# innnky/vispeech

Measured on AMD Instinct MI355X. Metric: 44.1kHz samples/sec, higher is better.
Workload: dtype f32 (split-f16 MFMA, 3-term); 1 GPU; C3: 64 mixed zh/ja utterances (~5 s each) per GPU, 44.1 kHz, hop 512, phoneme/duration/F0/energy/noise supplied, random-init (synthetic) weights of configs/config.json; 2 batches in flight per GPU; utterances_per_gpu=64, global_batch=64, padded_frames=489, frames_padded=31296, frames_computed=28902, parallelism=shard1, generator=f16s, controls=all, batches_in_flight=2

## Files before the change

vispeech_amd/csrc/api.hip:

```cpp
#include <algorithm>
#include <cmath>
#include <cstdlib>
#include <cstring>
#include <vector>

#include "model.h"

using namespace vsp;

namespace {

void generator_frame_dependence(const vsp_config& c, int resblock, int pre_k, int post_k, int& back, int& fwd);
long total_upsample(const vsp_config& c);

struct T3 {
  float* p = nullptr;
  long bs = 0, cs = 0;
  T3 chan(int c) const { return T3{p ? p + (size_t)c * cs : nullptr, bs, cs}; }
};

struct Ws {
  char* base;
  size_t cap;
  size_t cur = 0;
// ... 142 lines not shown
    if (prof) {
      const double in_el = (double)a.T_in * a.Cin, out_el = (double)(a.ups_s > 0 ? a.T_store * (a.M / a.ups_s) : a.Nq * a.M);
      const double ext = 4.0 * B * (in_el + out_el * (1.0 + (a.res ? 1.0 : 0.0) + (a.acc_prev ? 1.0 : 0.0)));
      prof_end(cls, 2.0 * a.M * a.Cin * a.K * (double)a.Nq * B, 4.0 * B * (in_el + out_el), ext, ext);
    }
  }
  void clconv(const ClConv& L, const float* x, float* out, const float* res, int T, bool acc_prev, float div, int B,
              const uint16_t* x_img = nullptr, uint16_t* o_img = nullptr) {
    if (dry() || !ok()) return;
    ClConvArgs a = L.phases > 1 ? cl_ups_args(cw(L), L.Cin, L.Cout, L.K, L.phases, x, T, CL_LRELU_SLOPE, out, terms())
                                : cl_conv_args(cw(L), L.Cin, L.Cout, L.K, L.dil, x, T, CL_LRELU_SLOPE, res, out, terms());
    a.x_img = x_img; a.o_img = o_img;
    a.acc_prev = acc_prev ? 1 : 0; a.div = div;
    a.glen = glen; a.g_in = L.phases > 1 ? grate_in : grate_out; a.g_store = grate_out;
    const bool prof = prof_begin(VSP_PROF_GENERATOR, fam(L.phases > 1 ? VSP_FAM_UPS : VSP_FAM_CONV, L.Cout));
    chk(launch_g16_conv(a, B, s), "g16_conv");
    if (prof) {
      const double in_el = (double)a.T_in * L.Cin, out_el = (double)a.T_store * L.Cout;
      const double ext = 4.0 * B * (in_el + out_el * (1.0 + (res ? 1.0 : 0.0) + (acc_prev ? 1.0 : 0.0)));
      prof_end(VSP_PROF_GENERATOR, 2.0 * L.Cout * L.Cin * L.K * L.phases * (double)a.Nq * B, 4.0 * B * (in_el + out_el), ext,
               ext + (out && o_img ? 4.0 * B * out_el : 0.0));
    }
  }
  void cond(const Conv& L, const float* g, float* out, int B) {
    const int gin = L.Cin;
    ConvArgs a = args(L, T3{const_cast<float*>(g), (long)gin, 1}, T3{out, (long)L.M, 1}, 1, 1);
    conv(a, B);
  }
  void ln(T3 x, T3 res, size_t gamma, size_t beta, T3 y, int B, int C, int T) {
    if (dry() || !ok()) return;
    chk(launch_layernorm(x.p, x.bs, x.cs, res.p, res.bs, res.cs, A(gamma), A(beta), y.p, y.bs, y.cs, B, C, T, s),
        "layernorm");
  }
};

void run_encoder_masked(Run& r, const EncoderW& E, int B, int T, T3 x_in, const int64_t* lengths, T3 y_out) {
  const vsp_config& c = r.ctx->cfg;
  const int h = c.hidden_channels, f = c.filter_channels;
  T3 X = r.ws.t3(B, h, T), S = r.ws.t3(B, h, T), QKV = r.ws.t3(B, 3 * h, T), AT = r.ws.t3(B, h, T),
     FF = r.ws.t3(B, f, T);
  void* AP = r.ctx->att_f16s ? r.ws.bytes(3 * attn_pack_bytes(B, c.n_heads, h / c.n_heads, T)) : nullptr;
  if (E.layers.empty()) {
    if (!r.dry() && r.ok()) {
      r.chk(launch_copy3(x_in.p, x_in.bs, x_in.cs, y_out.p, y_out.bs, y_out.cs, B, h, T, r.s), "copy");
      if (lengths) r.chk(launch_mask3(y_out.p, y_out.bs, y_out.cs, lengths, B, h, T, r.s), "mask");
    }
// ... 44 lines not shown
        }
      }
    } else {
      r.conv(a, B);
      r.ln(S, T3{}, L.g1, L.b1, X, B, h, T);
    }
    a = r.args(L.f1, X, FF, T, T);
    a.lengths = lengths; a.in_mask = 1; a.act = 1;
    r.conv(a, B);
    a = r.args(L.f2, FF, S, T, T);
    a.lengths = lengths; a.in_mask = 1; a.mask_pre = 1;
    a.res = X.p; a.r_bs = X.bs; a.r_cs = X.cs;
    r.conv(a, B);
    r.ln(S, T3{}, L.g2, L.b2, last ? y_out : X, B, h, T);
  }
  if (lengths && !r.dry() && r.ok()) r.chk(launch_mask3(y_out.p, y_out.bs, y_out.cs, lengths, B, h, T, r.s), "mask");
}

void mask3(Run& r, T3 x, const int64_t* lengths, int B, int C, int T) {
  if (r.dry() || !r.ok() || !lengths) return;
  r.chk(launch_mask3(x.p, x.bs, x.cs, lengths, B, C, T, r.s), "mask");
}

void run_wn(Run& r, const Conv* cond, const std::vector<Conv>& in, const std::vector<Conv>& res,
            const std::vector<Conv>& skip, int nl, int B, int T, T3 H, T3 ACT, T3 OUT, float* gc, long gc_bs, const float* g,
            const int64_t* lengths) {
  const int h = r.ctx->cfg.hidden_channels;
  if (cond) r.cond(*cond, g, gc, B);
  for (int l = 0; l < nl; ++l) {
    ConvArgs a = r.args(in[l], H, ACT, T, T);
    a.act = 2; a.cond = gc ? gc + (size_t)l * 2 * h : nullptr; a.cond_bs = gc_bs;
    r.conv(a, B);
    if (l < nl - 1) {
      a = r.args(res[l], ACT, H, T, T);
      a.res = H.p; a.r_bs = H.bs; a.r_cs = H.cs;
      a.lengths = lengths; a.mask_post = 1;
      a.split_row = h; a.out2 = OUT.p; a.o2_bs = OUT.bs; a.o2_cs = OUT.cs; a.acc_prev2 = l > 0;
      r.conv(a, B);
    } else {
      a = r.args(skip[l], ACT, OUT, T, T);
      a.acc_prev = l > 0;
      a.lengths = lengths; a.mask_post = 1;
      r.conv(a, B);
    }
  }
}

void run_flow(Run& r, int B, int T, T3 z, const float* g, const int64_t* lengths, bool reverse = true) {
  const vsp_config& c = r.ctx->cfg;
  const Model& m = r.ctx->model;
  const int h = c.hidden_channels, half = c.inter_channels / 2, fl = c.flow_layers;
  T3 H = r.ws.t3(B, h, T), ACT = r.ws.t3(B, h, T), OUT = r.ws.t3(B, h, T);
  const long gcs = (long)c.n_flows * 2 * h * fl;
  float* gc = r.ws.f((size_t)B * gcs);
  r.cond(m.flow_cond_all, g, gc, B);
  for (int n = 0; n < c.n_flows; ++n) {
    const int i = reverse ? c.n_flows - 1 - n : n;
    const FlowW& F = m.flows[i];
    const T3 x0 = F.flipped ? z.chan(half) : z;
    const T3 x1 = F.flipped ? z : z.chan(half);
    ConvArgs a = r.args(F.pre, x0, H, T, T);
    a.lengths = lengths; a.mask_post = 1;
    r.conv(a, B);
    run_wn(r, nullptr, F.in, F.res, F.skip, fl, B, T, H, ACT, OUT, gc ? gc + (size_t)i * 2 * h * fl : nullptr, gcs, g, lengths);
    a = r.args(F.post, OUT, x1, T, T);
    a.lengths = lengths; a.mask_pre = 1; a.alpha = reverse ? -1.f : 1.f;
    a.res = x1.p; a.r_bs = x1.bs; a.r_cs = x1.cs;
    a.mask_post = 1;
    r.conv(a, B);
  }
}

void run_posterior(Run& r, int B, int T, T3 y, const int64_t* lengths, const float* g, const float* noise, T3 Z,
                   T3 M, T3 LOGS) {
  const vsp_config& c = r.ctx->cfg;
  const PosteriorW& Q = r.ctx->model.enc_q;
  const int h = c.hidden_channels, ql = c.posterior_layers;
  T3 H = r.ws.t3(B, h, T), ACT = r.ws.t3(B, h, T), OUT = r.ws.t3(B, h, T);
  float* gc = r.ws.f((size_t)B * 2 * h * ql);
  if (r.dry()) return;
  ConvArgs a = r.args(Q.pre, y, H, T, T);
  a.lengths = lengths; a.mask_post = 1;
  r.conv(a, B);
  run_wn(r, &Q.cond, Q.in, Q.res, Q.skip, ql, B, T, H, ACT, OUT, gc, 2L * h * ql, g, lengths);
  a = r.args(Q.proj, OUT, M, T, T);
  a.lengths = lengths; a.mask_post = 1;
  a.split_row = c.inter_channels; a.out2 = LOGS.p; a.o2_bs = LOGS.bs; a.o2_cs = LOGS.cs; a.mask_post2 = 1;
  r.conv(a, B);
  if (r.ok()) {
    r.chk(launch_reparam(M.p, LOGS.p, noise, 1.f, Z.p, (long)B * c.inter_channels * T, r.s), "reparam");
    r.chk(launch_mask3(Z.p, Z.bs, Z.cs, lengths, B, c.inter_channels, T, r.s), "mask");
  }
}

template <class F>
size_t max_over_stages(const vsp_config& c, int T, size_t mx, F f) {
  long t = T;
  for (int i = 0; i < c.n_upsamples; ++i) {
    t *= c.upsample_rates[i];
    mx = std::max(mx, (size_t)f(c.upsample_initial_channel >> (i + 1), t));
  }
  return mx;
}

void run_generator(Run& r, int B, int T, T3 z, const int64_t* in_lengths, const float* g, float* o) {
  const vsp_config& c = r.ctx->cfg;
  const Model& m = r.ctx->model;
// ... 335 lines not shown
  if (!cfg || !out || (resblock != 1 && resblock != 2)) return VSP_ERR_ARG;
  vsp_ctx* ctx = new (std::nothrow) vsp_ctx();
  if (!ctx) return VSP_ERR_ARG;
  ctx->cfg = *cfg;
  ctx->resblock = resblock;
  ctx->device = device;
  if (const char* e = getenv("VSP_FRAME")) ctx->frame_f16s = strcmp(e, "f32") != 0;
  if (const char* e = getenv("VSP_ATT")) ctx->att_f16s = strcmp(e, "f32") != 0;
  bool want_f16 = false;
  if (const char* e = getenv("VSP_GENERATOR")) {
    if (!strcmp(e, "f32")) ctx->gen_mode = 0;
    want_f16 = !strcmp(e, "f16");
  }
  if (const char* e = getenv("VSP_FUSE_PAIRS")) ctx->fuse_pairs = atoi(e) != 0;
  if (const char* e = getenv("VSP_RB2_FUSE")) ctx->rb2_fuse = atoi(e) != 0;
  if (const char* e = getenv("VSP_TIMG")) ctx->t_img = atoi(e) != 0;
  if (const char* e = getenv("VSP_PP")) ctx->pp_pairs = atoi(e) != 0;
  if (const char* e = getenv("VSP_PAIR")) ctx->pair_ring = !strcmp(e, "ring");
  if (const char* e = getenv("VSP_CHAIN_RING")) ctx->chain_ring = atoi(e) != 0;
  if (const char* e = getenv("VSP_CHAIN")) ctx->chain_mask = atoi(e);
  if (const char* e = getenv("VSP_RW64")) ctx->rw64 = atoi(e) != 0;
  if (const char* e = getenv("VSP_TRIM_TAILS")) ctx->trim_tails = atoi(e) != 0;
  if (const char* e = getenv("VSP_COLS")) ctx->cols = atoi(e) != 0;
  if (const char* e = getenv("VSP_COLS_BLOCKS")) ctx->cols_blocks = atol(e);
  if (const char* e = getenv("VSP_COLS_MIN_BLOCKS")) ctx->cols_min_blocks = atol(e);
  if (const char* e = getenv("VSP_ACT_SCALE_LOG2")) {
    const int l = atoi(e);
    ctx->act_scale = std::ldexp(1.f, l < 0 ? 0 : l > 8 ? 8 : l);
  }
  if (const char* e = getenv("VSP_EARLY_FL")) ctx->early_fl = atoi(e) != 0;
  if (const char* e = getenv("VSP_RB_STREAMS")) ctx->rb_streams = atoi(e);
#ifdef VSP_EXPERIMENTS
  if (const char* e = getenv("VSP_ATT_KSPLIT")) ctx->att_ksplit = atoi(e);
  if (const char* e = getenv("VSP_CHUNK_MB")) ctx->chunk_mb = atof(e);
  if (const char* e = getenv("VSP_CHAIN_CH")) ctx->chain_ch = atoi(e);
  if (const char* e = getenv("VSP_CHAIN128")) ctx->chain128_mask = atoi(e);
#endif
  build_schema(ctx->cfg, ctx->schema, ctx->resblock);
  const int rc = plan_model(ctx);
  if (want_f16 && ctx->gen_mode == 1) ctx->gen_mode = 2;
  *out = ctx;
  return rc;
}

int vsp_destroy(vsp_ctx* ctx) {
  if (!ctx) return VSP_ERR_ARG;
// ... 615 lines not shown
  Run r{ctx, (hipStream_t)stream, ws};
  const long n = (long)B * ctx->cfg.inter_channels * Tf;
  r.chk(hipMemcpyAsync(z_p, z, n * sizeof(float), hipMemcpyDeviceToDevice, r.s), "z copy");
  run_flow(r, B, Tf, ext(z_p, ctx->cfg.inter_channels, Tf), g, frame_lengths, false);
  if (ws.overflow) return ctx->fail(VSP_ERR_WORKSPACE, "flow workspace too small (need %zu bytes)", ws.cur);
  return r.rc;
}

static int check_vc(vsp_ctx* ctx);

static int wn_layer_impl(vsp_ctx* ctx, hipStream_t s, Ws& ws, int which, int layer, int B, int T, float* x, const float* g,
                         const int64_t* lengths, float* skip, int accumulate) {
  const vsp_config& c = ctx->cfg;
  const Model& m = ctx->model;
  const int h = c.hidden_channels;
  const bool post = which < 0;
  const Conv& cond = post ? m.enc_q.cond : m.flows[which].cond;
  const std::vector<Conv>& in = post ? m.enc_q.in : m.flows[which].in;
  const std::vector<Conv>& res = post ? m.enc_q.res : m.flows[which].res;
  const std::vector<Conv>& sk = post ? m.enc_q.skip : m.flows[which].skip;
  const int nl = post ? c.posterior_layers : c.flow_layers;
  Run r{ctx, s, ws};
  T3 ACT = ws.t3(B, h, T);
  float* gc = ws.f((size_t)B * 2 * h * nl);
  if (ws.dry) return VSP_OK;
  if (ws.overflow) return ctx->fail(VSP_ERR_WORKSPACE, "wn layer workspace too small");
  const T3 H = ext(x, h, T), OUT = ext(skip, h, T);
  r.cond(cond, g, gc, B);
  ConvArgs a = r.args(in[layer], H, ACT, T, T);
  a.act = 2; a.cond = gc + (size_t)layer * 2 * h; a.cond_bs = 2L * h * nl;
  r.conv(a, B);
  if (layer < nl - 1) {
    a = r.args(res[layer], ACT, H, T, T);
    a.res = H.p; a.r_bs = H.bs; a.r_cs = H.cs;
    a.lengths = lengths; a.mask_post = 1;
    a.split_row = h; a.out2 = OUT.p; a.o2_bs = OUT.bs; a.o2_cs = OUT.cs; a.acc_prev2 = accumulate ? 1 : 0;
    r.conv(a, B);
  } else {
    a = r.args(sk[layer], ACT, OUT, T, T);
    a.acc_prev = accumulate ? 1 : 0;
    a.lengths = lengths; a.mask_post = 1;
    r.conv(a, B);
  }
  return r.rc;
}

int64_t vsp_wn_layer_workspace_bytes(const vsp_ctx* ctx, int which, int B, int T) {
  if (!ctx || B <= 0 || T <= 0 || which < -1 || which >= ctx->cfg.n_flows) return VSP_ERR_ARG;
  if (which < 0 && ctx->cfg.spec_channels <= 0) return VSP_ERR_ARG;
  Ws ws(nullptr, 0, true);
  wn_layer_impl(const_cast<vsp_ctx*>(ctx), nullptr, ws, which, 0, B, T, nullptr, nullptr, nullptr, nullptr, 0);
// ... 408 lines not shown
```

vispeech_amd/csrc/kernels.h:

```cpp
#pragma once
#include <hip/hip_runtime.h>
#include <stdint.h>

#include <atomic>

#include "../../include/vispeech_hip.h"

namespace vsp {

inline hipError_t set_max_dynamic_lds(const void* kern, int bytes, std::atomic<uint64_t>& done) {
  int dev = 0;
  hipError_t e = hipGetDevice(&dev);
  if (e != hipSuccess) return e;
  const uint64_t bit = 1ull << (dev & 63);
  if (done.load(std::memory_order_acquire) & bit) return hipSuccess;
  e = hipFuncSetAttribute(kern, hipFuncAttributeMaxDynamicSharedMemorySize, bytes);
  if (e == hipSuccess) done.fetch_or(bit, std::memory_order_release);
  return e;
}

constexpr int CONV_CK = 32;
constexpr int CONV_HALO = 64;

struct ConvArgs {
// ... 8 lines not shown
  int T_in;
  int Nq;
  int nchunks;
  int in_mask;
  int in_act; float in_slope;
  int act;
  int mask_pre;
  float alpha;
  int acc_prev;
  float div;
  int mask_post;
  int ups_s, ups_p, T_store;
  int f16s;
  int split_row; float* out2; long o2_bs, o2_cs; int acc_prev2;
  int mask_post2;
  const uint16_t* wg;
  long wg_min_blocks, wg_max_blocks;
};

hipError_t launch_conv(const ConvArgs& a, int B, hipStream_t s);
bool conv_cols_supported(const ConvArgs& a);
hipError_t launch_conv_cols(const ConvArgs& a, int B, hipStream_t s, const float* ln_gamma = nullptr,
                            const float* ln_beta = nullptr);
size_t packed_conv_floats(int M, int Cin, int K);
void pack_conv_weights(float* dst, int M, int Cin, int K, const float* dense );
void pack_conv_weights_f16s(float* dst, int M, int Cin, int K, const float* dense );

#ifndef G16_WSCALE_V
#define G16_WSCALE_V 256.f
#define G16_UNSCALE_V (1.f / 256.f)
#endif
constexpr float G16_WSCALE = G16_WSCALE_V, G16_UNSCALE = G16_UNSCALE_V;

#ifdef __HIPCC__
__device__ __forceinline__ void vsp_raise_flag(unsigned* flags, unsigned bit) {
  __hip_atomic_fetch_or(flags, bit, __ATOMIC_RELAXED, __HIP_MEMORY_SCOPE_SYSTEM);
}
#ifndef VSP_SPLIT_FORM
#define VSP_SPLIT_FORM 1
#endif
__device__ __forceinline__ void vsp_split_pair(float x0, float x1, unsigned& hi, unsigned& lo) {
#if VSP_SPLIT_FORM == 0
  const float h0 = __uint_as_float(__float_as_uint(x0) & 0xffffe000u), h1 = __uint_as_float(__float_as_uint(x1) & 0xffffe000u);
  float l0, l1;
  asm("v_sub_f32 %0, %1, %2" : "=v"(l0) : "v"(x0), "v"(h0));
  asm("v_sub_f32 %0, %1, %2" : "=v"(l1) : "v"(x1), "v"(h1));
// ... 188 lines not shown
```

vispeech_amd/csrc/model.h:

```cpp
#pragma once
#include <hip/hip_runtime.h>

#include <cstdarg>
#include <cstdio>
#include <map>
#include <string>
#include <vector>

#include "../../include/vispeech_hip.h"
#include "kernels.h"

namespace vsp {

struct HostTensor {
  std::vector<int64_t> shape;
  std::vector<float> data;
  size_t numel() const { size_t n = 1; for (auto s : shape) n *= (size_t)s; return n; }
};

struct Conv {
  int M = 0, Cin = 0, K = 1, dil = 1, pad = 0;
  int ups_s = 0, ups_p = 0;
  size_t w = 0;
  long b = -1;
  bool f16s = false;
  size_t wg = 0;
  bool has_wg = false;
};

struct ClConv {
  int Cout = 0, Cin = 0, K = 1, dil = 1, pad = 0, phases = 1, ups_p = 0;
  size_t wg = 0;
  long b = -1;
};

struct EncLayer {
  Conv qkv, o, f1, f2;
  size_t ek = 0, ev = 0, g1 = 0, b1 = 0, g2 = 0, b2 = 0;
};
struct EncoderW {
  std::string prefix;
  std::vector<EncLayer> layers;
};
struct FlowW {
  bool flipped = false;
  Conv pre, cond, post;
  std::vector<Conv> in, res, skip;
};
struct PosteriorW {
  Conv pre, cond, proj;
// ... 47 lines not shown
}

struct vsp_ctx {
  vsp_config cfg;
  int resblock = 1;
  int device = 0;
  std::string err;
  std::map<std::string, vsp::SchemaEntry> schema;
  std::map<std::string, vsp::HostTensor> raw;
  vsp::Model model;
  float* arena = nullptr;
  bool arena_owned = false;
  bool ready = false;
  bool t_img = true;
  bool pp_pairs = true;
  bool pair_ring = false;
  bool chain_ring = false;
  bool rw64 = false;
  float act_scale = 16.f;
  unsigned* flags_host = nullptr;
  unsigned* flags_dev = nullptr;
  long cols_min_blocks = 32;
  long cols_blocks = 256;
  bool cols = true;
  bool trim_tails = true;
  int rb_streams = 0;
  bool early_fl = true;
  int64_t* fl_pinned = nullptr;
  int fl_cap = 0, fl_n = 0;
  hipEvent_t fl_ev = nullptr;
  const int64_t* fl_src = nullptr;
  std::vector<int64_t> fl_known;
  const int64_t* fl_known_src = nullptr;
  hipStream_t side[2] = {nullptr, nullptr};
  std::vector<hipEvent_t> sync_ev;
  float* out_tab = nullptr;
  int out_L = 0, out_M = 0, out_H = 0, out_J = 0, out_P = 0;
  int64_t noise_first = 0;
  bool adopted_pending = false;
  int gen_mode = 1;
  bool frame_f16s = true;
  bool att_f16s = true;
  int att_ksplit = -1;
  int chain_mask = 0x1;
  int chain128_mask = 0;
  int chain_ch = 32;
// ... 33 lines not shown
```

vispeech_amd/csrc/weights.cpp:

```cpp
#include <cmath>
#include <cstring>
#include <functional>

#include "model.h"

namespace vsp {

using Shape = std::vector<int64_t>;

static void add(std::map<std::string, SchemaEntry>& s, const std::string& k, Shape shape, bool used = true) {
  s[k] = SchemaEntry{std::move(shape), used, false};
}

static void schema_encoder(std::map<std::string, SchemaEntry>& s, const std::string& p, int n_layers,
                           const vsp_config& c) {
  const int64_t h = c.hidden_channels, f = c.filter_channels, k = c.kernel_size, dk = h / c.n_heads;
  for (int i = 0; i < n_layers; ++i) {
    const std::string a = p + ".attn_layers." + std::to_string(i);
    add(s, a + ".emb_rel_k", {1, 2 * c.window_size + 1, dk});
    add(s, a + ".emb_rel_v", {1, 2 * c.window_size + 1, dk});
    for (const char* nm : {"conv_q", "conv_k", "conv_v", "conv_o"}) {
      add(s, a + "." + nm + ".weight", {h, h, 1});
      add(s, a + "." + nm + ".bias", {h});
    }
// ... 129 lines not shown
  add(s, "pitch_prenet.bias", {h});
  add(s, "energy_prenet.weight", {h, 1, 3});
  add(s, "energy_prenet.bias", {h});
  add(s, "emb_g.weight", {c.n_speakers, gin});
}

struct Planner {
  size_t cur = 0;
  bool f16s = false;
  size_t raw(size_t n) {
    const size_t o = cur;
    cur += (n + 63) / 64 * 64;
    return o;
  }
  Conv conv(int M, int Cin, int K, int dil, int pad, bool bias) {
    Conv c;
    c.M = M; c.Cin = Cin; c.K = K; c.dil = dil; c.pad = pad;
    c.w = raw(packed_conv_floats(M, Cin, K));
    c.b = bias ? (long)raw((size_t)M) : -1;
    c.f16s = f16s;
    if (f16s && K == 1 && Cin % 32 == 0 && Cin <= 192 && M % 16 == 0 && M >= 64 && M <= 576) {
      c.wg = raw(packed_g16_halfs(M, Cin, 1) / 2);
      c.has_wg = true;
    }
    return c;
  }
  ClConv clconv(int Cout, int Cin, int K, int dil, int pad, int phases, int ups_p) {
    ClConv c;
    c.Cout = Cout; c.Cin = Cin; c.K = K; c.dil = dil; c.pad = pad; c.phases = phases; c.ups_p = ups_p;
    c.wg = raw((cl_is_c16(Cout, Cin, phases) ? packed_g16c16_halfs(K) : packed_g16_halfs(phases * Cout, Cin, K)) / 2);
    c.b = (long)raw((size_t)Cout);
    return c;
  }
};

static void plan_encoder(Planner& p, EncoderW& e, const std::string& prefix, int n_layers, const vsp_config& c) {
  const int h = c.hidden_channels, f = c.filter_channels, k = c.kernel_size, dk = h / c.n_heads;
  const int nrel = 2 * c.window_size + 1;
  e.prefix = prefix;
  e.layers.resize(n_layers);
  for (auto& L : e.layers) {
    L.qkv = p.conv(3 * h, h, 1, 1, 0, true);
    L.o = p.conv(h, h, 1, 1, 0, true);
    L.ek = p.raw((size_t)nrel * dk);
    L.ev = p.raw((size_t)nrel * dk);
    L.g1 = p.raw(h); L.b1 = p.raw(h);
// ... 42 lines not shown
  m.pit_cond = p.conv(h, gin, 1, 1, 0, true);
  m.pit_pw = p.raw(h); m.pit_pb = p.raw(1);
  const int e = c.energy_filter;
  m.en_cond = p.conv(h, gin, 1, 1, 0, true);
  m.en_c1 = p.conv(e, h, 3, 1, 1, true);
  m.en_c2 = p.conv(e, e, 3, 1, 1, true);
  m.en_g1 = p.raw(e); m.en_b1 = p.raw(e); m.en_g2 = p.raw(e); m.en_b2 = p.raw(e);
  m.en_lw = p.raw(e); m.en_lb = p.raw(1);
  m.ppre_w = p.raw((size_t)h * 3); m.ppre_b = p.raw(h);
  m.epre_w = p.raw((size_t)h * 3); m.epre_b = p.raw(h);
  m.proj = p.conv(2 * inter, h, 1, 1, 0, true);
  m.flows.resize(c.n_flows);
  const int half = inter / 2, fk = c.flow_kernel, fl = c.flow_layers;
  m.flow_cond_all = p.conv(c.n_flows * 2 * h * fl, gin, 1, 1, 0, true);
  for (int i = 0; i < c.n_flows; ++i) {
    FlowW& F = m.flows[i];
    F.flipped = ((c.n_flows - i) % 2) == 1;
    F.pre = p.conv(h, half, 1, 1, 0, true);
    F.cond = m.flow_cond_all;
    F.cond.M = 2 * h * fl;
    F.cond.w = m.flow_cond_all.w + (size_t)i * packed_conv_floats(2 * h * fl, gin, 1);
    F.cond.b = m.flow_cond_all.b + (long)i * 2 * h * fl;
    for (int l = 0; l < fl; ++l) {
      F.in.push_back(p.conv(2 * h, h, fk, 1, (fk - 1) / 2, true));
      if (l < fl - 1) F.res.push_back(p.conv(2 * h, h, 1, 1, 0, true));
      F.skip.push_back(p.conv(h, h, 1, 1, 0, true));
    }
    F.post = p.conv(half, h, 1, 1, 0, true);
  }
  if (c.n_flows % 2)
    return ctx->fail(VSP_ERR_UNSUPPORTED, "odd n_flows leaves the latent channel-flipped; only even counts are folded");
  if (c.spec_channels > 0) {
    if (c.posterior_layers < 1) return ctx->fail(VSP_ERR_ARG, "posterior_layers < 1");
    const int n_fft = 2 * (c.spec_channels - 1);
    m.stft = p.conv(2 * c.spec_channels, n_fft, 1, 1, 0, false);
    PosteriorW& Q = m.enc_q;
    const int ql = c.posterior_layers;
    Q.pre = p.conv(h, c.spec_channels, 1, 1, 0, true);
    Q.cond = p.conv(2 * h * ql, gin, 1, 1, 0, true);
    for (int l = 0; l < ql; ++l) {
      Q.in.push_back(p.conv(2 * h, h, fk, 1, (fk - 1) / 2, true));
      if (l < ql - 1) Q.res.push_back(p.conv(2 * h, h, 1, 1, 0, true));
      Q.skip.push_back(p.conv(h, h, 1, 1, 0, true));
    }
    Q.proj = p.conv(2 * inter, h, 1, 1, 0, true);
  }
  const int c0 = c.upsample_initial_channel;
  int ch = c0;
  m.has_cl = true;
  for (int i = 0; i < c.n_upsamples; ++i) {
    const int cin = c0 >> i, cout = c0 >> (i + 1);
    const bool last16 = i == c.n_upsamples - 1 && cin == 32 && cout == 16 && c.upsample_rates[i] > 0 &&
                        (c.upsample_rates[i] * 16) % 32 == 0;
    if (last16) continue;
    if (cin % 32 || cout % 32 || (cin != 32 && cin % 64) || (cout != 32 && cout % 64)) m.has_cl = false;
  }
  if ((c0 >> c.n_upsamples) > 64)
    return ctx->fail(VSP_ERR_UNSUPPORTED, "conv_post kernels cover <= 64 input channels (got %d)", c0 >> c.n_upsamples);
  if (!m.has_cl) ctx->gen_mode = 0;
  p.f16s = ctx->frame_f16s && ctx->gen_mode != 0;
  m.g_pre = p.conv(c0, inter, 7, 1, 3, true);
  m.g_cond = p.conv(c0, gin, 1, 1, 0, true);
  p.f16s = false;
  for (int i = 0; i < c.n_upsamples; ++i) {
// ... 173 lines not shown
}

static void fill_wn(Filler& f, const std::string& p, const Conv& cond, const std::vector<Conv>& in,
                    const std::vector<Conv>& res, const std::vector<Conv>& skip, int nl, int h, int gin, int fk) {
  {
    const HostTensor* W = f.get(p + ".cond_layer.weight");
    const HostTensor* B = f.get(p + ".cond_layer.bias");
    if (!f.ok) return;
    const float* wd = W->data.data();
    const float* bd = B->data.data();
    auto orig = [=](int r) { return (r / (2 * h)) * 2 * h + gate_row(r % (2 * h), h); };
    f.conv(cond, [=](int r, int ci, int) { return wd[(size_t)orig(r) * gin + ci]; },
           [=](int r) { return bd[orig(r)]; });
  }
  for (int l = 0; l < nl && f.ok; ++l) {
    const std::string il = p + ".in_layers." + std::to_string(l);
    const HostTensor* W = f.get(il + ".weight");
    const HostTensor* B = f.get(il + ".bias");
    if (!f.ok) return;
    const float* wd = W->data.data();
    const float* bd = B->data.data();
    f.conv(in[l], [=](int r, int ci, int t) { return wd[((size_t)gate_row(r, h) * h + ci) * fk + t]; },
           [=](int r) { return bd[gate_row(r, h)]; });
    const std::string rs = p + ".res_skip_layers." + std::to_string(l);
    if (l < nl - 1) {
      f.conv_plain(res[l], rs + ".weight", rs + ".bias", 0);
      f.conv_plain(skip[l], rs + ".weight", rs + ".bias", h);
    } else {
      f.conv_plain(skip[l], rs + ".weight", rs + ".bias", 0);
    }
  }
}

int fill_model(vsp_ctx* ctx, std::vector<float>& arena) {
  const vsp_config& c = ctx->cfg;
  Model& m = ctx->model;
  arena.assign(m.total_floats, 0.f);
  Filler f{ctx, arena};
  const int h = c.hidden_channels, gin = c.gin_channels, inter = c.inter_channels;
  f.copy_raw(m.emb_sym, "enc_p.symbol_emb.weight", (size_t)c.n_vocab * h);
  f.copy_raw(m.emb_g, "emb_g.weight", (size_t)c.n_speakers * gin);
  for (int i = 0; i < 3; ++i) fill_encoder(f, m.enc[i], c);
  f.conv_plain(m.dur_cond, "duration_predictor.cond.weight", "duration_predictor.cond.bias");
  f.conv_plain(m.dur_c1, "duration_predictor.conv_1.weight", "duration_predictor.conv_1.bias");
  f.conv_plain(m.dur_c2, "duration_predictor.conv_2.weight", "duration_predictor.conv_2.bias");
  f.copy_raw(m.dur_g1, "duration_predictor.norm_1.gamma", c.dur_filter);
// ... 135 lines not shown
```

Before: 200.7 million samples/s.

## Fuse WaveNet in-conv, gated activation and res/skip conv into one kernel

```diff
diff --git a/vispeech_amd/csrc/api.hip b/vispeech_amd/csrc/api.hip
--- a/vispeech_amd/csrc/api.hip
+++ b/vispeech_amd/csrc/api.hip
@@ -188,6 +188,29 @@
                ext + (out && o_img ? 4.0 * B * out_el : 0.0));
     }
   }
+  void wn_layer(const Conv& in, const Conv& rs, T3 H, T3 H2, T3 OUT, const float* gc, long gc_bs, const int64_t* lengths, int T,
+                int B, bool acc) {
+    if (dry() || !ok()) return;
+    WnLayerArgs a;
+    std::memset(&a, 0, sizeof a);
+    a.h_in = H.p; a.h_bs = H.bs; a.h_cs = H.cs;
+    a.h_out = H2.p; a.ho_bs = H2.bs; a.ho_cs = H2.cs;
+    a.out = OUT.p; a.o_bs = OUT.bs; a.o_cs = OUT.cs;
+    a.w_in = reinterpret_cast<const uint16_t*>(A(in.wl)); a.b_in = A((size_t)in.b);
+    a.gc = gc; a.gc_bs = gc_bs;
+    a.w_rs = reinterpret_cast<const uint16_t*>(A(rs.wg)); a.b_rs = A((size_t)rs.b); a.rows_rs = rs.M;
+    a.lengths = lengths; a.T = T; a.acc = acc ? 1 : 0;
+    const bool prof = prof_begin(VSP_PROF_FRAME);
+    chk(launch_wn_layer(a, B, ctx->wn_tile, s), "wn_layer_f16s");
+    if (prof) {
+      const int h = in.Cin;
+      const bool last = rs.M == h;
+      const double el = (double)T * h, ac = acc ? 1.0 : 0.0;
+      const double bytes = 4.0 * B * el * (3.0 + 1.0 + rs.M / (double)h);
+      prof_end(VSP_PROF_FRAME, 2.0 * (2.0 * h * h * in.K + (double)rs.M * h) * (double)T * B, bytes,
+               bytes + 4.0 * B * el * ((last ? 0.0 : 1.0) + ac), 4.0 * B * el * ((last ? 2.0 : 3.0) + ac));
+    }
+  }
   void cond(const Conv& L, const float* g, float* out, int B) {
     const int gin = L.Cin;
     ConvArgs a = args(L, T3{const_cast<float*>(g), (long)gin, 1}, T3{out, (long)L.M, 1}, 1, 1);
@@ -278,11 +301,29 @@
   r.chk(launch_mask3(x.p, x.bs, x.cs, lengths, B, C, T, r.s), "mask");
 }
 
+bool wn_fused(const vsp_ctx* ctx, const std::vector<Conv>& in, const std::vector<Conv>& res, const std::vector<Conv>& skip, int nl,
+              int B, int T) {
+  if (!ctx->wn_fuse || !ctx->frame_f16s || nl < 1) return false;
+  const int h = ctx->cfg.hidden_channels;
+  for (int l = 0; l < nl; ++l) {
+    const Conv& rs = l < nl - 1 ? res[l] : skip[l];
+    if (!in[l].has_wl || !rs.has_wg || !wn_layer_supported(h, in[l].K, in[l].dil, rs.M, in[l].f16s && rs.f16s, true)) return false;
+  }
+  return (long)B * ((T + ctx->wn_tile - 1) / ctx->wn_tile) >= ctx->wn_min_blocks;
+}
+
 void run_wn(Run& r, const Conv* cond, const std::vector<Conv>& in, const std::vector<Conv>& res,
-            const std::vector<Conv>& skip, int nl, int B, int T, T3 H, T3 ACT, T3 OUT, float* gc, long gc_bs, const float* g,
+            const std::vector<Conv>& skip, int nl, int B, int T, T3 H, T3 H2, T3 ACT, T3 OUT, float* gc, long gc_bs, const float* g,
             const int64_t* lengths) {
   const int h = r.ctx->cfg.hidden_channels;
   if (cond) r.cond(*cond, g, gc, B);
+  if (H2.p && wn_fused(r.ctx, in, res, skip, nl, B, T)) {
+    for (int l = 0; l < nl; ++l) {
+      r.wn_layer(in[l], l < nl - 1 ? res[l] : skip[l], H, H2, OUT, gc ? gc + (size_t)l * 2 * h : nullptr, gc_bs, lengths, T, B, l > 0);
+      std::swap(H, H2);
+    }
+    return;
+  }
   for (int l = 0; l < nl; ++l) {
     ConvArgs a = r.args(in[l], H, ACT, T, T);
     a.act = 2; a.cond = gc ? gc + (size_t)l * 2 * h : nullptr; a.cond_bs = gc_bs;
@@ -307,6 +348,7 @@
   const Model& m = r.ctx->model;
   const int h = c.hidden_channels, half = c.inter_channels / 2, fl = c.flow_layers;
   T3 H = r.ws.t3(B, h, T), ACT = r.ws.t3(B, h, T), OUT = r.ws.t3(B, h, T);
+  const T3 H2 = r.ctx->wn_fuse ? r.ws.t3(B, h, T) : T3{};
   const long gcs = (long)c.n_flows * 2 * h * fl;
   float* gc = r.ws.f((size_t)B * gcs);
   r.cond(m.flow_cond_all, g, gc, B);
@@ -318,7 +360,7 @@
     ConvArgs a = r.args(F.pre, x0, H, T, T);
     a.lengths = lengths; a.mask_post = 1;
     r.conv(a, B);
-    run_wn(r, nullptr, F.in, F.res, F.skip, fl, B, T, H, ACT, OUT, gc ? gc + (size_t)i * 2 * h * fl : nullptr, gcs, g, lengths);
+    run_wn(r, nullptr, F.in, F.res, F.skip, fl, B, T, H, H2, ACT, OUT, gc ? gc + (size_t)i * 2 * h * fl : nullptr, gcs, g, lengths);
     a = r.args(F.post, OUT, x1, T, T);
     a.lengths = lengths; a.mask_pre = 1; a.alpha = reverse ? -1.f : 1.f;
     a.res = x1.p; a.r_bs = x1.bs; a.r_cs = x1.cs;
@@ -333,12 +375,13 @@
   const PosteriorW& Q = r.ctx->model.enc_q;
   const int h = c.hidden_channels, ql = c.posterior_layers;
   T3 H = r.ws.t3(B, h, T), ACT = r.ws.t3(B, h, T), OUT = r.ws.t3(B, h, T);
+  const T3 H2 = r.ctx->wn_fuse ? r.ws.t3(B, h, T) : T3{};
   float* gc = r.ws.f((size_t)B * 2 * h * ql);
   if (r.dry()) return;
   ConvArgs a = r.args(Q.pre, y, H, T, T);
   a.lengths = lengths; a.mask_post = 1;
   r.conv(a, B);
-  run_wn(r, &Q.cond, Q.in, Q.res, Q.skip, ql, B, T, H, ACT, OUT, gc, 2L * h * ql, g, lengths);
+  run_wn(r, &Q.cond, Q.in, Q.res, Q.skip, ql, B, T, H, H2, ACT, OUT, gc, 2L * h * ql, g, lengths);
   a = r.args(Q.proj, OUT, M, T, T);
   a.lengths = lengths; a.mask_post = 1;
   a.split_row = c.inter_channels; a.out2 = LOGS.p; a.o2_bs = LOGS.bs; a.o2_cs = LOGS.cs; a.mask_post2 = 1;
@@ -720,6 +763,9 @@
   if (const char* e = getenv("VSP_RW64")) ctx->rw64 = atoi(e) != 0;
   if (const char* e = getenv("VSP_TRIM_TAILS")) ctx->trim_tails = atoi(e) != 0;
   if (const char* e = getenv("VSP_COLS")) ctx->cols = atoi(e) != 0;
+  if (const char* e = getenv("VSP_WN_FUSE")) ctx->wn_fuse = atoi(e) != 0;
+  if (const char* e = getenv("VSP_WN_TILE")) ctx->wn_tile = atoi(e) == 64 ? 64 : 128;
+  if (const char* e = getenv("VSP_WN_MIN_BLOCKS")) ctx->wn_min_blocks = atol(e);
   if (const char* e = getenv("VSP_COLS_BLOCKS")) ctx->cols_blocks = atol(e);
   if (const char* e = getenv("VSP_COLS_MIN_BLOCKS")) ctx->cols_min_blocks = atol(e);
   if (const char* e = getenv("VSP_ACT_SCALE_LOG2")) {
@@ -1381,11 +1427,19 @@
   const int nl = post ? c.posterior_layers : c.flow_layers;
   Run r{ctx, s, ws};
   T3 ACT = ws.t3(B, h, T);
+  const T3 H2 = ctx->wn_fuse ? ws.t3(B, h, T) : T3{};
   float* gc = ws.f((size_t)B * 2 * h * nl);
   if (ws.dry) return VSP_OK;
   if (ws.overflow) return ctx->fail(VSP_ERR_WORKSPACE, "wn layer workspace too small");
   const T3 H = ext(x, h, T), OUT = ext(skip, h, T);
   r.cond(cond, g, gc, B);
+  if (H2.p && wn_fused(ctx, in, res, sk, nl, B, T)) {
+    const bool last = layer == nl - 1;
+    r.wn_layer(in[layer], last ? sk[layer] : res[layer], H, H2, OUT, gc + (size_t)layer * 2 * h, 2L * h * nl, lengths, T, B,
+               accumulate != 0);
+    if (!last && r.ok()) r.chk(launch_copy3(H2.p, H2.bs, H2.cs, H.p, H.bs, H.cs, B, h, T, s), "copy");
+    return r.rc;
+  }
   ConvArgs a = r.args(in[layer], H, ACT, T, T);
   a.act = 2; a.cond = gc + (size_t)layer * 2 * h; a.cond_bs = 2L * h * nl;
   r.conv(a, B);
diff --git a/vispeech_amd/csrc/kernels.h b/vispeech_amd/csrc/kernels.h
--- a/vispeech_amd/csrc/kernels.h
+++ b/vispeech_amd/csrc/kernels.h
@@ -54,6 +54,24 @@
 bool conv_cols_supported(const ConvArgs& a);
 hipError_t launch_conv_cols(const ConvArgs& a, int B, hipStream_t s, const float* ln_gamma = nullptr,
                             const float* ln_beta = nullptr);
+struct WnLayerArgs {
+  const float* h_in; long h_bs, h_cs;
+  float* h_out; long ho_bs, ho_cs;
+  float* out; long o_bs, o_cs;
+  const uint16_t* w_in;
+  const float* b_in;
+  const float* gc; long gc_bs;
+  const uint16_t* w_rs;
+  const float* b_rs;
+  int rows_rs;
+  const int64_t* lengths;
+  int T;
+  int acc;
+};
+bool wn_layer_supported(int h, int K, int dil, int rows_rs, bool f16s, bool images);
+hipError_t launch_wn_layer(const WnLayerArgs& a, int B, int tile , hipStream_t s);
+size_t packed_wn_in_halfs();
+void pack_wn_in_weights(uint16_t* dst, const float* dense );
 size_t packed_conv_floats(int M, int Cin, int K);
 void pack_conv_weights(float* dst, int M, int Cin, int K, const float* dense );
 void pack_conv_weights_f16s(float* dst, int M, int Cin, int K, const float* dense );
diff --git a/vispeech_amd/csrc/model.h b/vispeech_amd/csrc/model.h
--- a/vispeech_amd/csrc/model.h
+++ b/vispeech_amd/csrc/model.h
@@ -26,6 +26,8 @@
   bool f16s = false;
   size_t wg = 0;
   bool has_wg = false;
+  size_t wl = 0;
+  bool has_wl = false;
 };
 
 struct ClConv {
@@ -119,6 +121,9 @@
   unsigned* flags_dev = nullptr;
   long cols_min_blocks = 32;
   long cols_blocks = 256;
+  bool wn_fuse = true;
+  int wn_tile = 128;
+  long wn_min_blocks = 0;
   bool cols = true;
   bool trim_tails = true;
   int rb_streams = 0;
diff --git a/vispeech_amd/csrc/weights.cpp b/vispeech_amd/csrc/weights.cpp
--- a/vispeech_amd/csrc/weights.cpp
+++ b/vispeech_amd/csrc/weights.cpp
@@ -175,6 +175,14 @@
     if (f16s && K == 1 && Cin % 32 == 0 && Cin <= 192 && M % 16 == 0 && M >= 64 && M <= 576) {
       c.wg = raw(packed_g16_halfs(M, Cin, 1) / 2);
       c.has_wg = true;
+    }
+    return c;
+  }
+  Conv wn_in(int h, int K) {
+    Conv c = conv(2 * h, h, K, 1, (K - 1) / 2, true);
+    if (wn_layer_supported(h, K, 1, 2 * h, f16s, true)) {
+      c.wl = raw(packed_wn_in_halfs() / 2);
+      c.has_wl = true;
     }
     return c;
   }
@@ -263,7 +271,7 @@
     F.cond.w = m.flow_cond_all.w + (size_t)i * packed_conv_floats(2 * h * fl, gin, 1);
     F.cond.b = m.flow_cond_all.b + (long)i * 2 * h * fl;
     for (int l = 0; l < fl; ++l) {
-      F.in.push_back(p.conv(2 * h, h, fk, 1, (fk - 1) / 2, true));
+      F.in.push_back(p.wn_in(h, fk));
       if (l < fl - 1) F.res.push_back(p.conv(2 * h, h, 1, 1, 0, true));
       F.skip.push_back(p.conv(h, h, 1, 1, 0, true));
     }
@@ -280,7 +288,7 @@
     Q.pre = p.conv(h, c.spec_channels, 1, 1, 0, true);
     Q.cond = p.conv(2 * h * ql, gin, 1, 1, 0, true);
     for (int l = 0; l < ql; ++l) {
-      Q.in.push_back(p.conv(2 * h, h, fk, 1, (fk - 1) / 2, true));
+      Q.in.push_back(p.wn_in(h, fk));
       if (l < ql - 1) Q.res.push_back(p.conv(2 * h, h, 1, 1, 0, true));
       Q.skip.push_back(p.conv(h, h, 1, 1, 0, true));
     }
@@ -500,6 +508,7 @@
     const float* bd = B->data.data();
     f.conv(in[l], [=](int r, int ci, int t) { return wd[((size_t)gate_row(r, h) * h + ci) * fk + t]; },
            [=](int r) { return bd[gate_row(r, h)]; });
+    if (in[l].has_wl && f.ok) pack_wn_in_weights(reinterpret_cast<uint16_t*>(f.arena.data() + in[l].wl), wd);
     const std::string rs = p + ".res_skip_layers." + std::to_string(l);
     if (l < nl - 1) {
       f.conv_plain(res[l], rs + ".weight", rs + ".bias", 0);
diff --git a/vispeech_amd/csrc/wn_fused.hip b/vispeech_amd/csrc/wn_fused.hip
--- /dev/null
+++ b/vispeech_amd/csrc/wn_fused.hip
@@ -0,0 +1,270 @@
+#include "g16_common.h"
+
+#include <cstring>
+#include <vector>
+
+namespace vsp {
+
+constexpr int WNF_H = 192, WNF_K = 5, WNF_NC = WNF_H / 32;
+constexpr int WNF_SLOT = 16384, WNF_NS = 3;
+constexpr int WNF_SUB_IN = WNF_NC * WNF_K * 3, WNF_SUB = WNF_SUB_IN + WNF_NC * 3;
+
+inline constexpr int wnf_plane_bytes(int W) { return (W + WNF_K - 1) * 16; }
+inline constexpr int wnf_window_bytes(int W) { return WNF_NC * 8 * wnf_plane_bytes(W); }
+inline constexpr int wnf_lds_bytes(int W) { return wnf_window_bytes(W) + WNF_NS * WNF_SLOT + 3 * 2 * WNF_H * 4; }
+
+size_t packed_wn_in_halfs() { return packed_g16_halfs(2 * WNF_H, WNF_H, WNF_K); }
+
+void pack_wn_in_weights(uint16_t* dst, const float* dense) {
+  std::vector<float> perm((size_t)2 * WNF_H * WNF_H * WNF_K);
+  for (int pr = 0; pr < 2 * WNF_H; ++pr) {
+    const int j = pr / 32, within = pr % 32;
+    const int row = within < 16 ? 16 * j + within : WNF_H + 16 * j + (within - 16);
+    std::memcpy(perm.data() + (size_t)pr * WNF_H * WNF_K, dense + (size_t)row * WNF_H * WNF_K, sizeof(float) * WNF_H * WNF_K);
+  }
+  pack_g16_weights(dst, 2 * WNF_H, WNF_H, WNF_K, perm.data());
+}
+
+template <int W, bool LAST>
+__global__ void __launch_bounds__(512, 2) wn_layer_f16s(WnLayerArgs a) {
+  constexpr int NW = W / 32;
+  constexpr int WR = W + WNF_K - 1, PL = WR * 16, CHB = 8 * PL, XSZ = WNF_NC * CHB;
+  constexpr int MT = LAST ? 1 : 2;
+  extern __shared__ __attribute__((aligned(16))) char lds[];
+  char* const X = lds;
+  char* const Rg = lds + XSZ;
+  float* const par = reinterpret_cast<float*>(lds + XSZ + WNF_NS * WNF_SLOT);
+
+  const int tid = threadIdx.x;
+  const int wave = __builtin_amdgcn_readfirstlane(tid >> 6);
+  const int lane = tid & 63, q = lane >> 4, l15 = lane & 15;
+  const int wm = wave >> 1, wn = wave & 1;
+  const int b = blockIdx.y, t0 = blockIdx.x * W, T = a.T;
+  int len = T;
+  if (a.lengths) { const long l = a.lengths[b]; len = l < 0 ? 0 : (l < T ? (int)l : T); }
+
+  const uint4* const Win = reinterpret_cast<const uint4*>(a.w_in);
+  const uint4* const Wrs = reinterpret_cast<const uint4*>(a.w_rs);
+  auto dma = [&](int i, int slot) {
+    const uint4* src;
+    if (i < WNF_SUB_IN) {
+      const int step = i / 3, p = i - 3 * step;
+      src = Win + ((size_t)(step * 24 + 6 * wm + 2 * p) * 2 + 2 * wn) * 64;
+    } else {
+      const int j = i - WNF_SUB_IN, c = j / 3, p = j - 3 * c;
+      src = LAST ? Wrs + ((size_t)(c * 12 + 3 * wm + p) * 2) * 64 : Wrs + ((size_t)(c * 24 + 6 * wm + 2 * p) * 2 + 2 * wn) * 64;
+    }
+    char* const dst = Rg + slot * WNF_SLOT + wm * 4096 + wn * 2048;
+    __builtin_amdgcn_global_load_lds((const __attribute__((address_space(1))) void*)(src + lane),
+                                     (__attribute__((address_space(3))) void*)dst, 16, 0, 0);
+    __builtin_amdgcn_global_load_lds((const __attribute__((address_space(1))) void*)(src + 64 + lane),
+                                     (__attribute__((address_space(3))) void*)(dst + 1024), 16, 0, 0);
+  };
+  dma(0, 0);
+  dma(1, 1);
+
+  for (int i = tid; i < 2 * WNF_H; i += 512) {
+    par[i] = a.b_in[i];
+    par[2 * WNF_H + i] = a.gc ? a.gc[(size_t)b * a.gc_bs + i] : 0.f;
+    par[4 * WNF_H + i] = i < a.rows_rs ? a.b_rs[i] : 0.f;
+  }
+
+  {
+    constexpr int UNITS = (WNF_H / 8) * WR, ITER = (UNITS + 511) / 512;
+    const float* const hb = a.h_in + (size_t)b * a.h_bs;
+    float v[ITER][8];
+#pragma unroll
+    for (int it = 0; it < ITER; ++it) {
+      const int u = tid + 512 * it, grp = u / WR, r = u - grp * WR, col = t0 - (WNF_K - 1) / 2 + r;
+      const bool in = u < UNITS && col >= 0 && col < T;
+      const float* xp = hb + (in ? (long)grp * 8 * a.h_cs + col : 0);
+#pragma unroll
+      for (int j = 0; j < 8; ++j) v[it][j] = in ? xp[(long)j * a.h_cs] : 0.f;
+    }
+#pragma unroll
+    for (int it = 0; it < ITER; ++it) {
+      const int u = tid + 512 * it, grp = u / WR, r = u - grp * WR;
+      if (u < UNITS) {
+        unsigned hi[4], lo[4];
+#pragma unroll
+        for (int j = 0; j < 4; ++j) vsp_split_pair(v[it][2 * j], v[it][2 * j + 1], hi[j], lo[j]);
+        const int c = grp >> 2, q4 = grp & 3;
+        *reinterpret_cast<u32x4*>(X + ((c * 2 + 0) * 4 + q4) * PL + r * 16) = u32x4{hi[0], hi[1], hi[2], hi[3]};
+        *reinterpret_cast<u32x4*>(X + ((c * 2 + 1) * 4 + q4) * PL + r * 16) = u32x4{lo[0], lo[1], lo[2], lo[3]};
+      }
+    }
+  }
+
+  const unsigned lds0 = (unsigned)(uintptr_t)(__attribute__((address_space(3))) char*)lds;
+  const unsigned a_lane = lds0 + XSZ + wm * 4096 + lane * 16;
+  const unsigned xb0 = lds0 + q * PL + (wn * (W / 2) + l15) * 16;
+  f16x8 Ah[2][2], Al[2][2], Bh[NW], Bl[NW];
+  f32x4 acc[6][NW];
+
+  auto read_a = [&](auto PP, auto SL, auto NMC) {
+    constexpr int pp = decltype(PP)::value, sl = decltype(SL)::value;
+    Ah[pp][0] = g16_lds_read<sl * WNF_SLOT>(a_lane);
+    Al[pp][0] = g16_lds_read<sl * WNF_SLOT + 1024>(a_lane);
+    if constexpr (decltype(NMC)::value == 2) {
+      Ah[pp][1] = g16_lds_read<sl * WNF_SLOT + 2048>(a_lane);
+      Al[pp][1] = g16_lds_read<sl * WNF_SLOT + 3072>(a_lane);
+    }
+  };
+  auto read_b = [&](auto J, unsigned addr) {
+    constexpr int j = decltype(J)::value;
+    Bh[j] = g16_lds_read<j * 256>(addr);
+    Bl[j] = g16_lds_read<j * 256 + 4 * PL>(addr);
+  };
+  auto substep = [&](auto KK, auto NMC, int i, unsigned b_next) {
+    constexpr int k = decltype(KK)::value, p = k % 3, pp = k & 1, NM = decltype(NMC)::value;
+    g16_vmcnt<0>();
+    G16_BARRIER();
+    if (i + 2 < WNF_SUB) dma(i + 2, (k + 2) % 3);
+    read_a(std::integral_constant<int, 1 - pp>{}, std::integral_constant<int, (k + 1) % 3>{}, NMC);
+    g16_lgkmcnt<2 * NM>();
+    g16_for<NW>([&](auto J) {
+      constexpr int j = decltype(J)::value;
+      __builtin_amdgcn_sched_barrier(0);
+      g16_for<NM>([&](auto I) {
+        constexpr int m = decltype(I)::value;
+        acc[NM * p + m][j] = G16_MFMA(Ah[pp][m], Bh[j], acc[NM * p + m][j]);
+        acc[NM * p + m][j] = G16_MFMA(Al[pp][m], Bh[j], acc[NM * p + m][j]);
+        acc[NM * p + m][j] = G16_MFMA(Ah[pp][m], Bl[j], acc[NM * p + m][j]);
+      });
+      __builtin_amdgcn_sched_barrier(0);
+      if constexpr (p == 2) read_b(J, b_next);
+    });
+  };
+  auto drain = [&]() {
+    g16_lgkmcnt<0>();
+    __builtin_amdgcn_sched_barrier(0);
+#pragma unroll
+    for (int m = 0; m < 2; ++m) asm volatile("" ::"v"(Ah[0][m]), "v"(Ah[1][m]), "v"(Al[0][m]), "v"(Al[1][m]));
+#pragma unroll
+    for (int j = 0; j < NW; ++j) asm volatile("" ::"v"(Bh[j]), "v"(Bl[j]));
+  };
+  using I0 = std::integral_constant<int, 0>; using I1 = std::integral_constant<int, 1>; using I2 = std::integral_constant<int, 2>;
+  using I3 = std::integral_constant<int, 3>; using I4 = std::integral_constant<int, 4>; using I5 = std::integral_constant<int, 5>;
+
+#pragma unroll
+  for (int m = 0; m < 6; ++m)
+#pragma unroll
+    for (int j = 0; j < NW; ++j) acc[m][j] = f32x4{0.f, 0.f, 0.f, 0.f};
+  g16_vmcnt<0>();
+  G16_BARRIER();
+  read_a(I0{}, I0{}, I2{});
+  g16_for<NW>([&](auto J) { read_b(J, xb0); });
+  for (int s = 0; s < WNF_NC * WNF_K; s += 2) {
+    const int s1 = s + 1, s2 = s + 2 < WNF_NC * WNF_K ? s + 2 : s + 1;
+    const unsigned b1 = xb0 + (s1 / WNF_K) * CHB + (s1 % WNF_K) * 16, b2 = xb0 + (s2 / WNF_K) * CHB + (s2 % WNF_K) * 16;
+    substep(I0{}, I2{}, 3 * s, b1); substep(I1{}, I2{}, 3 * s + 1, b1); substep(I2{}, I2{}, 3 * s + 2, b1);
+    substep(I3{}, I2{}, 3 * s + 3, b2); substep(I4{}, I2{}, 3 * s + 4, b2); substep(I5{}, I2{}, 3 * s + 5, b2);
+  }
+  drain();
+  G16_BARRIER();
+
+#pragma unroll
+  for (int p = 0; p < 3; ++p) {
+    const int j = 3 * wm + p, r0 = 16 * j + 4 * q;
+    const int it = 64 * (r0 >> 5) + (r0 & 31);
+    const f32x4 bt = *reinterpret_cast<const f32x4*>(par + it), bs = *reinterpret_cast<const f32x4*>(par + it + 32);
+    const f32x4 ct = *reinterpret_cast<const f32x4*>(par + 2 * WNF_H + it), cs = *reinterpret_cast<const f32x4*>(par + 2 * WNF_H + it + 32);
+    char* const dst = X + ((j >> 1) * 8 + 2 * (j & 1) + (q >> 1)) * PL + (wn * (W / 2) + l15) * 16 + 8 * (q & 1);
+#pragma unroll
+    for (int n = 0; n < NW; ++n) {
+      const f32x4 va = (acc[2 * p][n] * G16_UNSCALE + bt) + ct, vb = (acc[2 * p + 1][n] * G16_UNSCALE + bs) + cs;
+      float v[4];
+#pragma unroll
+      for (int r = 0; r < 4; ++r) v[r] = tanhf(va[r]) * (1.f / (1.f + expf(-vb[r])));
+      unsigned hi[2], lo[2];
+      vsp_split_pair(v[0], v[1], hi[0], lo[0]);
+      vsp_split_pair(v[2], v[3], hi[1], lo[1]);
+      *reinterpret_cast<u32x2*>(dst + n * 256) = u32x2{hi[0], hi[1]};
+      *reinterpret_cast<u32x2*>(dst + n * 256 + 4 * PL) = u32x2{lo[0], lo[1]};
+    }
+  }
+#pragma unroll
+  for (int m = 0; m < 6; ++m)
+#pragma unroll
+    for (int j = 0; j < NW; ++j) acc[m][j] = f32x4{0.f, 0.f, 0.f, 0.f};
+  G16_BARRIER();
+
+  g16_for<NW>([&](auto J) { read_b(J, xb0); });
+  using NMT = std::integral_constant<int, MT>;
+  for (int c = 0; c < WNF_NC; c += 2) {
+    const int i = WNF_SUB_IN + 3 * c;
+    const unsigned b1 = xb0 + (c + 1) * CHB, b2 = xb0 + (c + 2 < WNF_NC ? c + 2 : c + 1) * CHB;
+    substep(I0{}, NMT{}, i, b1); substep(I1{}, NMT{}, i + 1, b1); substep(I2{}, NMT{}, i + 2, b1);
+    substep(I3{}, NMT{}, i + 3, b2); substep(I4{}, NMT{}, i + 4, b2); substep(I5{}, NMT{}, i + 5, b2);
+  }
+  drain();
+
+  constexpr int NM = 6 / (LAST ? 2 : 1);
+  const int row0 = 16 * NM * wm;
+  const bool to_h = !LAST && wm < 2;
+  const int drow = (!LAST && !to_h) ? row0 - WNF_H : row0;
+  float* const dstb = to_h ? a.h_out + (size_t)b * a.ho_bs + (long)drow * a.ho_cs : a.out + (size_t)b * a.o_bs + (long)drow * a.o_cs;
+  const long dcs = to_h ? a.ho_cs : a.o_cs;
+  const float* const srcb = to_h ? a.h_in + (size_t)b * a.h_bs + (long)drow * a.h_cs : (a.acc ? dstb : nullptr);
+  const long scs = to_h ? a.h_cs : a.o_cs;
+  const bool masked = LAST || to_h;
+  const float* const bias = par + 4 * WNF_H + row0;
+  f32x4 sv[NM][NW];
+#pragma unroll
+  for (int m = 0; m < NM; ++m)
+#pragma unroll
+    for (int n = 0; n < NW; ++n) sv[m][n] = f32x4{0.f, 0.f, 0.f, 0.f};
+  if (srcb) {
+#pragma unroll
+    for (int m = 0; m < NM; ++m)
+#pragma unroll
+      for (int n = 0; n < NW; ++n) {
+        const int col = t0 + wn * (W / 2) + 16 * n + l15;
+        if (col < T) {
+#pragma unroll
+          for (int r = 0; r < 4; ++r) sv[m][n][r] = srcb[(long)(16 * m + 4 * q + r) * scs + col];
+        }
+      }
+  }
+#pragma unroll
+  for (int m = 0; m < NM; ++m) {
+    const f32x4 bv = *reinterpret_cast<const f32x4*>(bias + 16 * m + 4 * q);
+#pragma unroll
+    for (int n = 0; n < NW; ++n) {
+      const int col = t0 + wn * (W / 2) + 16 * n + l15;
+      f32x4 v = acc[m][n] * G16_UNSCALE + bv;
+      v += sv[m][n];
+      if (masked && col >= len) v = f32x4{0.f, 0.f, 0.f, 0.f};
+      if (col < T) {
+#pragma unroll
+        for (int r = 0; r < 4; ++r) dstb[(long)(16 * m + 4 * q + r) * dcs + col] = v[r];
+      }
+    }
+  }
+}
+
+bool wn_layer_supported(int h, int K, int dil, int rows_rs, bool f16s, bool images) {
+  return f16s && images && h == WNF_H && K == WNF_K && dil == 1 && (rows_rs == WNF_H || rows_rs == 2 * WNF_H);
+}
+
+template <int W, bool LAST>
+static hipError_t launch_wn_tile(const WnLayerArgs& a, int B, hipStream_t s) {
+  constexpr int lds = wnf_lds_bytes(W);
+  static_assert(lds <= 160 * 1024, "LDS budget");
+  static std::atomic<uint64_t> attr_done{0};
+  auto kern = wn_layer_f16s<W, LAST>;
+  if (hipError_t e = set_max_dynamic_lds(reinterpret_cast<const void*>(kern), lds, attr_done); e != hipSuccess) return e;
+  hipLaunchKernelGGL(kern, dim3((a.T + W - 1) / W, B), dim3(512), lds, s, a);
+  return hipGetLastError();
+}
+
+hipError_t launch_wn_layer(const WnLayerArgs& a, int B, int tile, hipStream_t s) {
+  const bool last = a.rows_rs == WNF_H;
+  if (!wn_layer_supported(WNF_H, WNF_K, 1, a.rows_rs, true, a.w_in && a.w_rs) || B <= 0 || B > 65535 || a.T <= 0 || !a.h_in ||
+      !a.out || !a.b_in || !a.b_rs || (!last && (!a.h_out || a.h_out == a.h_in)) || (tile != 64 && tile != 128))
+    return hipErrorInvalidValue;
+  if (tile == 64) return last ? launch_wn_tile<64, true>(a, B, s) : launch_wn_tile<64, false>(a, B, s);
+  return last ? launch_wn_tile<128, true>(a, B, s) : launch_wn_tile<128, false>(a, B, s);
+}
+
+}
```

New measurement: 201.2 million samples/s (median of 6 runs). About the same (+0.3%).
